# fpgasystems/GPU-FPGA-Recommendation-System

Measured on AMD Instinct MI355X. Metric: inferences/sec at batch 256, higher is better.
Workload: dtype f32; 1 GPU; Model-A (embedding_47_krnl: 47 tables, 1.415 GB) batch=256, fp32 FC 352-1024-512-256-1, all tables resident in one GPU's HBM; hash-filled tables, uniform per-table indices; index rows resident in HBM when the timed region starts (1024 rotating buffers), scores left in HBM (the bench contract's definition of `value`); value_pcie_inclusive = the reference's own loop (cuda_server.c:460-461,494-495): ; batch=256, driver_threads=2, workers_per_thread=2, batches_per_launch=64, parallelism=replicas x1

## Files before the change

### gpu-fpga-recommendation-system_amd/csrc/fr_fused.hip

```cpp
#include "fr_device.h"

#ifdef FR_EPI_FORMS
#include <cstdarg>
#include <cstdio>
thread_local char fr_epi_noted[96];
thread_local int fr_epi_hip_error = 0;
void fr_set_error(const char *, ...) {}
void fr_note_kernel(const char *fmt, ...) {
    va_list ap;
    va_start(ap, fmt);
    vsnprintf(fr_epi_noted, sizeof(fr_epi_noted), fmt, ap);
    va_end(ap);
}
#define FR_NO_DEFAULT_FORM() return FR_ERR_INVALID
#else
static int fused_epi_forward(const FrFusedArgs &a, int kind, hipStream_t s) {
    char name[96] = "";
    const int e = fr_epi_fused_launch(&a, kind, s, name, sizeof(name));
    if (e) FR_FAIL(FR_ERR_HIP, "launch of the epilogue form of the fused kernel failed: %s", hipGetErrorString((hipError_t)e));
    fr_note_kernel("%s", name);
    return FR_OK;
}
#endif

// ... 307 lines not shown
        stamp();
        if (c == 1) wstamp(1);
        ft_gemm_ct<T2W, RB, 32>(acc2, ring2, W2, 32 * T2W * wave, R1, 0, 32 * c, hk, lm);
        if (c == 1) wstamp(2);
        if constexpr (KG > 0) {
            const int cn = (c + 1 < n_chunks) ? c + 1 : c;
            ft_ring_fill<1, RA, KG1>(ring1, W1, cn * 256 + 32 * wave, 0);
        }
    }
    float4 ring3[RA][1];
    ft_ring_fill<1, RA, 32 * T2W>(ring3, W3, 32 * wave, 0);
    __syncthreads();
#pragma unroll
    for (int t = 0; t < T2W; t++) ft_store_tile<EPI>(R2, acc2[t], 32 * (T2W * wave + t), hk, lm, a.epi[1], 32 * (T2W * wave + t));
    __syncthreads();
    stamp();

    f32x16 acc3[1];
#pragma unroll
    for (int i = 0; i < 16; i++) acc3[0][i] = 0.0f;
    ft_gemm_ct<1, RA, 32 * T2W>(acc3, ring3, W3, 32 * wave, R2, 0, 0, hk, lm);
    if (!DB) __syncthreads();
    ft_store_tile<EPI>(R3, acc3[0], 32 * wave, hk, lm, a.epi[2], 32 * wave);
    __syncthreads();
    stamp();
    {
        const int il = tid & 31, sl = tid >> 5;
        const int rows_per = (a.H3 / 4) / 16;
        float s = 0.0f;
        for (int q = sl * rows_per; q < (sl + 1) * rows_per; q++) {
            const uint4 r = R3[(size_t)q * FR_FT_LD + il];
            const float4 w4 = reinterpret_cast<const float4 *>(a.wout)[q];
            s = fmaf(w4.x, __uint_as_float(r.x), s);
            s = fmaf(w4.y, __uint_as_float(r.y), s);
            s = fmaf(w4.z, __uint_as_float(r.z), s);
            s = fmaf(w4.w, __uint_as_float(r.w), s);
        }
        float *part = reinterpret_cast<float *>(R3 + (size_t)64 * FR_FT_LD);
        part[sl * 32 + il] = s;
        __syncthreads();
        if (tid < 32 && m0 + tid < bt.batch) {
            float t = part[tid];
#pragma unroll
            for (int i = 1; i < 16; i++) t += part[i * 32 + tid];
            t = ft_out_bias<EPI>(a, t);
            bt.scores[m0 + tid] = t;
        }
    }
    stamp();
}

#ifndef FR_EPI_FORMS
template <int T2W, int KG, int WPE, bool DB>
__global__ void __launch_bounds__(512, WPE) fr_fused_tile_kernel(const FrFusedArgs a) {
    fused_tile_body<T2W, KG, WPE, DB, false>(a);
}
#else
template <int T2W, int KG, int WPE, bool DB>
__global__ void __launch_bounds__(512, WPE) fr_epi_tile_kernel(const FrFusedArgs a) {
    fused_tile_body<T2W, KG, WPE, DB, true>(a);
}
#endif

size_t frk_fused_lds_bytes(int K, int H2, int wpe) {
    if (wpe == 4) {
        const size_t phase1 = (size_t)(K / 4) + 64, phase2 = (size_t)(H2 / 4) > 68 ? (size_t)(H2 / 4) : 68;
        return (phase1 > phase2 ? phase1 : phase2) * FR_FT_LD * 16;
    }
    const size_t phase1 = (size_t)(K / 4) + 128;
    const size_t phase2 = (size_t)(H2 / 4) + 64 + 4;
    return (phase1 > phase2 ? phase1 : phase2) * FR_FT_LD * 16;
}

bool frk_fused_ok(int K, int H1, int H2, int H3) {
    const bool straight = (K == 352 || K == 880) && H2 == 512;
    if ((!straight && K % 32) || H1 % 256 || (H2 != 256 && H2 != 512) || H3 != 256) return false;
    return frk_fused_lds_bytes(K, H2, 4) <= 160 * 1024;
}

static int fused_wpe(int K, int H2) {
#ifdef FR_EXPERIMENTS
    const int forced = FR_KNOB_ONCE("FUSED_WPE", 0);
    if (forced == 2 || forced == 4) return forced == 4 && frk_fused_lds_bytes(K, H2, 4) > 80 * 1024 ? 2 : forced;
#endif
    return frk_fused_lds_bytes(K, H2, 4) <= 80 * 1024 ? 4 : 2;
}

#ifndef FR_EPI_FORMS
template <int T2W, int KG, int WPE, bool DB>
static int fused_launch_inst(const FrFusedArgs &a, dim3 grid, size_t lds, hipStream_t s) {
    static FrLdsAttrOnce lds_once;
    if (int rc_ = fr_allow_full_lds(&fr_fused_tile_kernel<T2W, KG, WPE, DB>, lds_once)) return rc_;
    fr_fused_tile_kernel<T2W, KG, WPE, DB><<<grid, dim3(512), lds, s>>>(a);
    fr_note_kernel("fr_fused_tile_kernel<%d, %d, %d, %s>", T2W, KG, WPE, DB ? "true" : "false");
    KCHECK();
    return FR_OK;
}

#else
template <int T2W, int KG, int WPE, bool DB>
static int fused_launch_epi_inst(const FrFusedArgs &a, dim3 grid, size_t lds, hipStream_t s) {
    static FrLdsAttrOnce lds_once;
    if (int rc_ = fr_allow_full_lds(&fr_epi_tile_kernel<T2W, KG, WPE, DB>, lds_once)) return rc_;
    fr_epi_tile_kernel<T2W, KG, WPE, DB><<<grid, dim3(512), lds, s>>>(a);
    fr_note_kernel("fr_epi_tile_kernel<%d, %d, %d, %s>", T2W, KG, WPE, DB ? "true" : "false");
    KCHECK();
    return FR_OK;
}

#endif
static bool fused_has_epi(const FrFusedArgs &a) { return a.epi[3].bias != nullptr; }

int frk_fused_launch(const FrFusedArgs &a, hipStream_t s) {
    const int wpe = fused_wpe(a.K, a.H2);
    (void)wpe;
    dim3 grid(a.n_batches * a.tiles_per_batch);
    if (fused_has_epi(a)) {
#ifndef FR_EPI_FORMS
        return fused_epi_forward(a, FR_EPI_KIND_F32, s);
#else
        if (a.H2 == 512 && a.K == 352) return fused_launch_epi_inst<2, 44, 2, true>(a, grid, frk_fused_lds_bytes(a.K, a.H2, 2), s);
        const bool db = frk_fused_lds_bytes(a.K, a.H2, 4) > 80 * 1024 && frk_fused_lds_bytes(a.K, a.H2, 2) <= 160 * 1024;
        const size_t lds = frk_fused_lds_bytes(a.K, a.H2, db ? 2 : 4);
        if (a.H2 == 512) {
            if (a.K == 880) return fused_launch_epi_inst<2, 110, 2, false>(a, grid, lds, s);
            return db ? fused_launch_epi_inst<2, 0, 2, true>(a, grid, lds, s) : fused_launch_epi_inst<2, 0, 2, false>(a, grid, lds, s);
        }
        return db ? fused_launch_epi_inst<1, 0, 2, true>(a, grid, lds, s) : fused_launch_epi_inst<1, 0, 2, false>(a, grid, lds, s);
#endif
    }
#ifdef FR_EPI_FORMS
    FR_NO_DEFAULT_FORM();
#else
    const bool db = wpe == 2 && frk_fused_lds_bytes(a.K, a.H2, 2) <= 160 * 1024;
    const size_t lds = frk_fused_lds_bytes(a.K, a.H2, db ? 2 : 4);
    if (a.H2 == 512) {
        if (a.K == 352) {
#ifdef FR_EXPERIMENTS
            if (wpe != 4) return fused_launch_inst<2, 44, 2, true>(a, grid, lds, s);
#endif
            return fused_launch_inst<2, 44, 4, false>(a, grid, lds, s);
        }
        if (a.K == 880) return fused_launch_inst<2, 110, 2, false>(a, grid, lds, s);
        if (db) return fused_launch_inst<2, 0, 2, true>(a, grid, lds, s);
        return fused_launch_inst<2, 0, 2, false>(a, grid, lds, s);
    }
    if (db) return fused_launch_inst<1, 0, 2, true>(a, grid, lds, s);
    return fused_launch_inst<1, 0, 2, false>(a, grid, lds, s);
#endif
}

constexpr int FR_M2_LD = 65;

template <int NT, int MT, int R, int CNT, int GA, int GB>
__device__ __forceinline__ void ftm_gemm_seg(f32x16 (&acc)[NT][MT], f32x16 (&alt)[MT], float4 (&ring)[R][NT], const FtW &w, int n0, const uint4 *Bq, int gb0,
                                             int g0, int hk, int lm) {
    const unsigned s0 = (unsigned)g0 * w.row2 + (unsigned)n0 * 16u;
    const uint4 *bl = Bq + (size_t)(2 * gb0 + hk) * FR_M2_LD + lm;
    uint4 bcur[MT];
#pragma unroll
    for (int mt = 0; mt < MT; mt++) bcur[mt] = bl[(size_t)(2 * GA) * FR_M2_LD + 32 * mt];
#pragma unroll
    for (int g = GA; g < GB; g++) {
        uint4 bnext[MT];
        const int gn = (g + 1 < GB) ? g + 1 : g;
#pragma unroll
        for (int mt = 0; mt < MT; mt++) bnext[mt] = bl[(size_t)(2 * gn) * FR_M2_LD + 32 * mt];
        const float4(&a4)[NT] = ring[g % R];
#pragma unroll
        for (int c = 0; c < 4; c++)
#pragma unroll
            for (int t = 0; t < NT; t++)
#pragma unroll
                for (int mt = 0; mt < MT; mt++) {
                    const float av = c == 0 ? a4[t].x : c == 1 ? a4[t].y : c == 2 ? a4[t].z : a4[t].w;
                    const uint32_t bv = c == 0 ? bcur[mt].x : c == 1 ? bcur[mt].y : c == 2 ? bcur[mt].z : bcur[mt].w;
                    if (NT == 1 && (c & 1)) alt[mt] = __builtin_amdgcn_mfma_f32_32x32x2f32(av, __uint_as_float(bv), alt[mt], 0, 0, 0);
                    else acc[t][mt] = __builtin_amdgcn_mfma_f32_32x32x2f32(av, __uint_as_float(bv), acc[t][mt], 0, 0, 0);
                }
        if (g + R < CNT) {
#pragma unroll
            for (int t = 0; t < NT; t++) ring[g % R][t] = ft_wload(w, s0 + (unsigned)(g + R) * w.row2, 512 * t);
        }
        __builtin_amdgcn_sched_barrier(0);
#pragma unroll
        for (int mt = 0; mt < MT; mt++) bcur[mt] = bnext[mt];
    }
}

template <int NT, int MT>
__device__ __forceinline__ void ftm_alt_zero(f32x16 (&alt)[MT]) {
    if constexpr (NT == 1) {
#pragma unroll
        for (int mt = 0; mt < MT; mt++)
#pragma unroll
            for (int i = 0; i < 16; i++) alt[mt][i] = 0.0f;
    }
}
template <int NT, int MT>
__device__ __forceinline__ void ftm_alt_add(f32x16 (&acc)[NT][MT], const f32x16 (&alt)[MT]) {
    if constexpr (NT == 1) {
#pragma unroll
        for (int mt = 0; mt < MT; mt++)
#pragma unroll
            for (int i = 0; i < 16; i++) acc[0][mt][i] += alt[mt][i];
    }
}

template <int NT, int MT, int R, int CNT>
__device__ __forceinline__ void ftm_gemm_ct(f32x16 (&acc)[NT][MT], float4 (&ring)[R][NT], const FtW &w, int n0, const uint4 *Bq, int gb0, int g0, int hk,
                                            int lm) {
    f32x16 alt[MT];
    ftm_alt_zero<NT, MT>(alt);
    ftm_gemm_seg<NT, MT, R, CNT, 0, CNT>(acc, alt, ring, w, n0, Bq, gb0, g0, hk, lm);
    ftm_alt_add<NT, MT>(acc, alt);
}

template <bool EPI>
__device__ __forceinline__ void ftm_store_tile(uint4 *img, const f32x16 &acc, int n_local, int m_local, int hk, int lm, const FrEpi &e, int n_glob) {
#pragma unroll
    for (int i = 0; i < 4; i++) {
        float c0 = acc[4 * i + 0], c1 = acc[4 * i + 1], c2 = acc[4 * i + 2], c3 = acc[4 * i + 3];
        ft_epi4<EPI>(c0, c1, c2, c3, e, n_glob + 8 * i, hk);
        uint4 v;
        v.x = __float_as_uint(c0);
        v.y = __float_as_uint(c1);
        v.z = __float_as_uint(c2);
        v.w = __float_as_uint(c3);
        img[(size_t)((n_local >> 2) + 2 * i + hk) * FR_M2_LD + m_local + lm] = v;
    }
}

template <int W0, int W>
struct FtmSlot {
    static constexpr int IPT = W / 8;
    uint64_t base;
    uint32_t stride, rows, icol;
    bool dense;
    uint32_t id[IPT];
    uint4 v[IPT];
    static __device__ __forceinline__ int word(int lane) { return W0 + (lane & (W - 1)); }
    static __device__ __forceinline__ int item(int lane, int wave, int i) { return lane / W + (64 / W) * (wave + 8 * i); }
    __device__ __forceinline__ void desc(const FrFusedArgs &a, const FrFusedBatch &bt, int lane) {
        const int w = word(lane) < a.n_words ? word(lane) : a.n_words - 1;
        const uint4 d0 = reinterpret_cast<const uint4 *>(a.words)[2 * w];
        const uint4 d1 = reinterpret_cast<const uint4 *>(a.words)[2 * w + 1];
        dense = (d0.w & FR_DESC_DENSE) != 0;
        base = (dense ? (uint64_t)reinterpret_cast<uintptr_t>(bt.dense) : 0ull) + (((uint64_t)d0.y << 32) | d0.x);
        stride = d0.z, rows = d1.x, icol = dense ? 0u : d0.w * 4u;
    }
    __device__ __forceinline__ void index(const FrFusedArgs &a, const __amdgpu_buffer_rsrc_t &rs_idx, int m0, int lane, int wave) {
#pragma unroll
        for (int i = 0; i < IPT; i++)
            id[i] = (uint32_t)__builtin_amdgcn_raw_buffer_load_b32(rs_idx, (unsigned)(m0 + item(lane, wave, i)) * (unsigned)a.idx_stride * 4u + icol, 0, 0);
    }
    __device__ __forceinline__ bool check(const FrFusedBatch &bt, int m0, int lane, int wave) {
        bool bad = false;
#pragma unroll
        for (int i = 0; i < IPT; i++) {
            const unsigned m = (unsigned)(m0 + item(lane, wave, i));
            uint32_t r = id[i];
            const bool oob = !dense & (r >= rows);
            bad |= oob;
            r = oob ? 0u : r;
            id[i] = dense ? (m < (unsigned)bt.batch ? m : 0u) : r;
        }
        return bad;
    }
    __device__ __forceinline__ void load() {
#pragma unroll
        for (int i = 0; i < IPT; i++) {
            typedef const u32x4_t __attribute__((address_space(1))) * gptr_t;
            const u32x4_t q = *(gptr_t)(base + (uint64_t)id[i] * stride);
            v[i] = make_uint4(q.x, q.y, q.z, q.w);
        }
    }
    __device__ __forceinline__ void put(const FrFusedArgs &a, const FrFusedBatch &bt, uint4 *Xq, int m0, int lane, int wave) const {
        if (word(lane) < a.n_words) {
#pragma unroll
            for (int i = 0; i < IPT; i++) {
                const int it = item(lane, wave, i);
                Xq[(size_t)word(lane) * FR_M2_LD + it] = (m0 + it < bt.batch) ? v[i] : make_uint4(0u, 0u, 0u, 0u);
            }
        }
    }
};
template <class... S>
struct FtmSlice : S... {
    __device__ __forceinline__ void desc(const FrFusedArgs &a, const FrFusedBatch &bt, int lane) { (S::desc(a, bt, lane), ...); }
    __device__ __forceinline__ void index(const FrFusedArgs &a, const __amdgpu_buffer_rsrc_t &rs, int m0, int lane, int wave) { (S::index(a, rs, m0, lane, wave), ...); }
    __device__ __forceinline__ bool check(const FrFusedBatch &bt, int m0, int lane, int wave) { return (false | ... | S::check(bt, m0, lane, wave)); }
    __device__ __forceinline__ void load() { (S::load(), ...); }
    __device__ __forceinline__ void put(const FrFusedArgs &a, const FrFusedBatch &bt, uint4 *Xq, int m0, int lane, int wave) const { (S::put(a, bt, Xq, m0, lane, wave), ...); }
};
constexpr int FR_M2_CUT1 = 12, FR_M2_CUT2 = 28;
using FtmS0 = FtmSlice<FtmSlot<0, 16>, FtmSlot<16, 8>>;
using FtmS1 = FtmSlice<FtmSlot<24, 32>>;
using FtmS2 = FtmSlice<FtmSlot<56, 32>>;

template <int KG, bool EPI>
__device__ __forceinline__ void fused_tile_m2_body(const FrFusedArgs &a) {
    extern __shared__ uint4 lds[];
    constexpr int LD = FR_M2_LD, MT = 2, T2W = 2, TI = 64;
    constexpr int RA = 12, RB = 8, GC1 = FR_M2_CUT1, GC2 = FR_M2_CUT2;
    static_assert(KG == 44 && GC1 < GC2 && GC2 < KG, "the slices above are cut for 88 record words");
    const int KQ = a.K / 4;
    uint4 *Xq = lds;
    uint4 *R1 = Xq + (size_t)KQ * LD;
    uint4 *R2 = lds;
    uint4 *R3 = lds;
    const int tid = threadIdx.x, lane = tid & 63;
    const int wave = __builtin_amdgcn_readfirstlane(tid >> 6);
    const int hk = lane >> 5, lm = lane & 31;
    const int bi = blockIdx.x / a.tiles_per_batch, tile = blockIdx.x - bi * a.tiles_per_batch;
    const FrFusedBatch &bt = a.b[bi];
    const int m0 = tile * TI;
    if (m0 >= bt.batch) return;
    const FtW W1 = ft_w(a.w1q, a.K, a.H1, hk, lm), W2 = ft_w(a.w2q, a.H1, a.H2, hk, lm), W3 = ft_w(a.w3q, a.H2, a.H3, hk, lm);
    float4 ring1[RA][1];
    ft_ring_fill<1, RA, KG>(ring1, W1, 32 * wave, 0);

    FtmS0 s0;
    FtmS1 s1;
    FtmS2 s2;
    s0.desc(a, bt, lane), s1.desc(a, bt, lane), s2.desc(a, bt, lane);
    const __amdgpu_buffer_rsrc_t rs_idx = __builtin_amdgcn_make_buffer_rsrc(const_cast<int32_t *>(bt.idx), 0, (unsigned)bt.batch * (unsigned)a.idx_stride * 4u, 0x00020000);
    s0.index(a, rs_idx, m0, lane, wave), s1.index(a, rs_idx, m0, lane, wave), s2.index(a, rs_idx, m0, lane, wave);
    const bool bad0 = s0.check(bt, m0, lane, wave), bad1 = s1.check(bt, m0, lane, wave), bad2 = s2.check(bt, m0, lane, wave);
    s0.load(), s1.load();
    if (bad0 | bad1 | bad2) atomicOr_system(a.err_flag, 1);
    s0.put(a, bt, Xq, m0, lane, wave);
    __syncthreads();

    const int n_chunks = a.H1 / 256;
    f32x16 acc2[T2W][MT];
    auto fc2_chunk = [&](int c, f32x16(&acc1)[1][MT]) {
        float4 ring2[RB][T2W];
        ft_ring_fill<T2W, RB, 32>(ring2, W2, 32 * T2W * wave, 32 * c);
        if (c > 0) __syncthreads();
#pragma unroll
        for (int mt = 0; mt < MT; mt++) ftm_store_tile<EPI>(R1, acc1[0][mt], 32 * wave, 32 * mt, hk, lm, a.epi[0], c * 256 + 32 * wave);
        __syncthreads();
        ftm_gemm_ct<T2W, MT, RB, 32>(acc2, ring2, W2, 32 * T2W * wave, R1, 0, 32 * c, hk, lm);
        if constexpr (EPI) {
            const int cn = (c + 1 < n_chunks) ? c + 1 : c;
            ft_ring_fill<1, RA, KG>(ring1, W1, cn * 256 + 32 * wave, 0);
        } else {
            if (c + 1 < n_chunks) ft_ring_fill<1, RA, KG>(ring1, W1, (c + 1) * 256 + 32 * wave, 0);
            else ft_ring_fill<1, RA, 32 * T2W>(ring1, W3, 32 * wave, 0);
        }
    };
    {
        f32x16 acc1[1][MT], alt1[MT];
#pragma unroll
        for (int mt = 0; mt < MT; mt++)
#pragma unroll
            for (int i = 0; i < 16; i++) acc1[0][mt][i] = 0.0f;
        ftm_alt_zero<1, MT>(alt1);
        ftm_gemm_seg<1, MT, RA, KG, 0, GC1>(acc1, alt1, ring1, W1, 32 * wave, Xq, 0, 0, hk, lm);
        s1.put(a, bt, Xq, m0, lane, wave);
        __syncthreads();
        s2.load();
        ftm_gemm_seg<1, MT, RA, KG, GC1, GC2>(acc1, alt1, ring1, W1, 32 * wave, Xq, 0, 0, hk, lm);
        s2.put(a, bt, Xq, m0, lane, wave);
        __syncthreads();
        ftm_gemm_seg<1, MT, RA, KG, GC2, KG>(acc1, alt1, ring1, W1, 32 * wave, Xq, 0, 0, hk, lm);
        ftm_alt_add<1, MT>(acc1, alt1);
#pragma unroll
        for (int t = 0; t < T2W; t++)
#pragma unroll
            for (int mt = 0; mt < MT; mt++)
#pragma unroll
                for (int i = 0; i < 16; i++) acc2[t][mt][i] = 0.0f;
        fc2_chunk(0, acc1);
    }
    for (int c = 1; c < n_chunks; c++) {
        f32x16 acc1[1][MT];
#pragma unroll
        for (int mt = 0; mt < MT; mt++)
#pragma unroll
            for (int i = 0; i < 16; i++) acc1[0][mt][i] = 0.0f;
        ftm_gemm_ct<1, MT, RA, KG>(acc1, ring1, W1, c * 256 + 32 * wave, Xq, 0, 0, hk, lm);
        fc2_chunk(c, acc1);
    }
    float4(&ring3)[RA][1] = ring1;
    if constexpr (EPI) ft_ring_fill<1, RA, 32 * T2W>(ring3, W3, 32 * wave, 0);
    __syncthreads();
#pragma unroll
    for (int t = 0; t < T2W; t++)
#pragma unroll
        for (int mt = 0; mt < MT; mt++) ftm_store_tile<EPI>(R2, acc2[t][mt], 32 * (T2W * wave + t), 32 * mt, hk, lm, a.epi[1], 32 * (T2W * wave + t));
    __syncthreads();

    f32x16 acc3[1][MT];
#pragma unroll
    for (int mt = 0; mt < MT; mt++)
#pragma unroll
        for (int i = 0; i < 16; i++) acc3[0][mt][i] = 0.0f;
    ftm_gemm_ct<1, MT, RA, 32 * T2W>(acc3, ring3, W3, 32 * wave, R2, 0, 0, hk, lm);
    __syncthreads();
#pragma unroll
    for (int mt = 0; mt < MT; mt++) ftm_store_tile<EPI>(R3, acc3[0][mt], 32 * wave, 32 * mt, hk, lm, a.epi[2], 32 * wave);
    __syncthreads();
    {
        const int il = tid & 63, sg = tid >> 6;
        const int rows_per = (a.H3 / 4) / 16;
        float *part = reinterpret_cast<float *>(R3 + (size_t)(a.H3 / 4) * LD);
#pragma unroll
        for (int h2 = 0; h2 < 2; h2++) {
            const int sl = 2 * sg + h2;
            float s = 0.0f;
            for (int q = sl * rows_per; q < (sl + 1) * rows_per; q++) {
                const uint4 r = R3[(size_t)q * LD + il];
                const float4 w4 = reinterpret_cast<const float4 *>(a.wout)[q];
                s = fmaf(w4.x, __uint_as_float(r.x), s);
                s = fmaf(w4.y, __uint_as_float(r.y), s);
                s = fmaf(w4.z, __uint_as_float(r.z), s);
                s = fmaf(w4.w, __uint_as_float(r.w), s);
            }
            part[sl * 64 + il] = s;
        }
        __syncthreads();
        if (tid < 64 && m0 + tid < bt.batch) {
            float t = part[tid];
#pragma unroll
            for (int i = 1; i < 16; i++) t += part[i * 64 + tid];
            t = ft_out_bias<EPI>(a, t);
            bt.scores[m0 + tid] = t;
        }
    }
}

#ifndef FR_EPI_FORMS
template <int KG>
__global__ void __launch_bounds__(512) fr_fused_tile_m2_kernel(const FrFusedArgs a) {
    fused_tile_m2_body<KG, false>(a);
}
#else
template <int KG>
__global__ void __launch_bounds__(512) fr_epi_tile_m2_kernel(const FrFusedArgs a) {
    fused_tile_m2_body<KG, true>(a);
}
#endif

bool frk_fused_m2_ok(int K, int H1, int H2, int H3) { return K == 352 && H1 % 256 == 0 && H2 == 512 && H3 == 256; }

int frk_fused_m2_launch(const FrFusedArgs &a, hipStream_t s) {
    static FrLdsAttrOnce lds_once;
    const size_t rows1 = (size_t)(a.K / 4) + 64, rows2 = (size_t)(a.H2 / 4), rows3 = 64 + 4;
    const size_t rows = rows1 > rows2 ? (rows1 > rows3 ? rows1 : rows3) : (rows2 > rows3 ? rows2 : rows3);
#ifdef FR_EPI_FORMS
    if (!fused_has_epi(a)) FR_NO_DEFAULT_FORM();
    if (int rc_ = fr_allow_full_lds(&fr_epi_tile_m2_kernel<44>, lds_once)) return rc_;
    fr_epi_tile_m2_kernel<44><<<dim3(a.n_batches * a.tiles_per_batch), dim3(512), rows * FR_M2_LD * 16, s>>>(a);
    fr_note_kernel("fr_epi_tile_m2_kernel<44>");
#else
    if (fused_has_epi(a)) return fused_epi_forward(a, FR_EPI_KIND_F32_M2, s);
    if (int rc_ = fr_allow_full_lds(&fr_fused_tile_m2_kernel<44>, lds_once)) return rc_;
    fr_fused_tile_m2_kernel<44><<<dim3(a.n_batches * a.tiles_per_batch), dim3(512), rows * FR_M2_LD * 16, s>>>(a);
    fr_note_kernel("fr_fused_tile_m2_kernel<44>");
#endif
    KCHECK();
    return FR_OK;
}

template <int NT, int MT, int R, int CNT>
__device__ __forceinline__ void fth_gemm_ct(f32x16 (&acc)[NT][MT], const FtW &w, int n0, const uint4 *Bh, int ld, int gb0, int g0, int hk, int lm) {
    const unsigned s0 = (unsigned)g0 * w.row2 + (unsigned)n0 * 16u;
    const uint4 *bl = Bh + (size_t)(2 * gb0 + hk) * ld + lm;
    uint4 ring[R][NT];
#pragma unroll
    for (int g = 0; g < R && g < CNT; g++)
#pragma unroll
        for (int t = 0; t < NT; t++) ring[g][t] = __builtin_bit_cast(uint4, ft_wload(w, s0 + (unsigned)g * w.row2, 512 * t));
#pragma unroll
    for (int g = 0; g < CNT; g++) {
        uint4 b8[MT];
#pragma unroll
        for (int mt = 0; mt < MT; mt++) b8[mt] = bl[(size_t)(2 * g) * ld + 32 * mt];
#pragma unroll
        for (int t = 0; t < NT; t++)
#pragma unroll
            for (int mt = 0; mt < MT; mt++)
                acc[t][mt] = __builtin_amdgcn_mfma_f32_32x32x16_bf16(__builtin_bit_cast(bf16x8, ring[g % R][t]), __builtin_bit_cast(bf16x8, b8[mt]),
                                                                     acc[t][mt], 0, 0, 0);
        if (g + R < CNT) {
#pragma unroll
            for (int t = 0; t < NT; t++) ring[g % R][t] = __builtin_bit_cast(uint4, ft_wload(w, s0 + (unsigned)(g + R) * w.row2, 512 * t));
        }
        __builtin_amdgcn_sched_barrier(0);
    }
}

template <bool EPI>
__device__ __forceinline__ void fth_store_tile(uint4 *img, int ld, const f32x16 &acc, int n_local, int m_local, int hk, int lm, const FrEpi &e, int n_glob) {
    uint2 *h = reinterpret_cast<uint2 *>(img);
#pragma unroll
    for (int i = 0; i < 4; i++) {
        float c0 = acc[4 * i + 0], c1 = acc[4 * i + 1], c2 = acc[4 * i + 2], c3 = acc[4 * i + 3];
        ft_epi4<EPI>(c0, c1, c2, c3, e, n_glob + 8 * i, hk);
        uint2 v;
        v.x = pack_bf16x2(c0, c1);
        v.y = pack_bf16x2(c2, c3);
        h[((size_t)((n_local >> 3) + i) * ld + m_local + lm) * 2 + hk] = v;
    }
}

template <int MT, int T2W, int KG, bool DB, int RD, int PD, bool EPI>
__device__ __forceinline__ void fused_tile_h_body(const FrFusedArgs &a) {
    extern __shared__ uint4 lds[];
    constexpr int LD = 32 * MT + 1, TI = 32 * MT;
    const int KO = a.K / 8;
    uint4 *Xh = lds;
    uint4 *R1b[2] = {Xh + (size_t)KO * LD, Xh + (size_t)(KO + (DB ? 32 : 0)) * LD};
    uint4 *R2 = lds;
    uint4 *R3 = lds + (size_t)(a.H2 / 8) * LD;
    const int tid = threadIdx.x, lane = tid & 63;
    const int wave = __builtin_amdgcn_readfirstlane(tid >> 6);
    const int hk = lane >> 5, lm = lane & 31;
    const int bi = blockIdx.x / a.tiles_per_batch, tile = blockIdx.x - bi * a.tiles_per_batch;
    const FrFusedBatch &bt = a.b[bi];
    const int m0 = tile * TI;
    if (m0 >= bt.batch) return;
    int n_st = 0;
    auto stamp = [&]() {
        if (a.stamps && lane == 0 && n_st < 14) {
            a.stamps[16ull * (8ull * blockIdx.x + wave) + n_st] = __builtin_amdgcn_s_memrealtime();
            if (n_st == 1) a.stamps[16ull * (8ull * blockIdx.x + wave) + 14] = __builtin_amdgcn_s_memtime();
            if (n_st == 9) a.stamps[16ull * (8ull * blockIdx.x + wave) + 15] = __builtin_amdgcn_s_memtime();
        }
        n_st++;
    };
    stamp();

    {
        const int wl = tid & 63, ig = tid >> 6;
        constexpr int IPT = TI / 8, NB = (4 * KG + 63) / 64;
        uint2 *Xh2 = reinterpret_cast<uint2 *>(Xh);
        const bool bad = ft_gather_tile<NB, IPT>(a, bt, m0, wl, ig, [&](int w, int i, const uint4 &x) {
            uint2 hv;
            hv.x = pack_bf16x2(__uint_as_float(x.x), __uint_as_float(x.y));
            hv.y = pack_bf16x2(__uint_as_float(x.z), __uint_as_float(x.w));
            Xh2[((size_t)(w >> 1) * LD + IPT * ig + i) * 2 + (w & 1)] = hv;
        });
        if (bad) atomicOr_system(a.err_flag, 1);
    }
    __syncthreads();
    stamp();

    f32x16 acc2[T2W][MT];
#pragma unroll
    for (int t = 0; t < T2W; t++)
#pragma unroll
        for (int mt = 0; mt < MT; mt++)
#pragma unroll
            for (int i = 0; i < 16; i++) acc2[t][mt][i] = 0.0f;
    const int n_chunks = a.H1 / 256;
    const FtW W1 = ft_w(a.w1q, a.K / 2, a.H1, hk, lm), W2 = ft_w(a.w2q, a.H1 / 2, a.H2, hk, lm), W3 = ft_w(a.w3q, a.H2 / 2, a.H3, hk, lm);
    static_assert(T2W == 2 && KG >= RD && RD >= 8 && RD <= 32 && RD % 2 == 0, "the stream ring assumes two n tiles per wave in FC2 (32 elements per chunk) and at least RD k groups in FC1");
    constexpr int OFF2 = KG % RD;
    uint4 ring[RD];
    auto w1load = [&](int c, int g) { return __builtin_bit_cast(uint4, ft_wload(W1, (unsigned)g * W1.row2 + (unsigned)(c * 256 + 32 * wave) * 16u, 0)); };
    auto w2load = [&](int c, int e) {
        return __builtin_bit_cast(uint4, ft_wload(W2, (unsigned)(16 * c + (e >> 1)) * W2.row2 + (unsigned)(32 * T2W * wave) * 16u, 512 * (e & 1)));
    };
#pragma unroll
    for (int g = 0; g < RD; g++) ring[g] = w1load(0, g);
    const uint4 *blx = Xh + (size_t)hk * LD + lm;
    static_assert(PD == 1 || PD == 2 || PD == 4, "B ring: 16 % PD must be 0");
    uint4 bq[PD][MT];
#pragma unroll
    for (int i = 0; i < PD; i++)
#pragma unroll
        for (int mt = 0; mt < MT; mt++) bq[i][mt] = blx[(size_t)(2 * i) * LD + 32 * mt];
    for (int c = 0; c < n_chunks; c++) {
        f32x16 acc1[1][MT];
#pragma unroll
        for (int mt = 0; mt < MT; mt++)
#pragma unroll
            for (int i = 0; i < 16; i++) acc1[0][mt][i] = 0.0f;
#pragma unroll
        for (int g = 0; g < KG; g++) {
#pragma unroll
// ... 376 lines not shown
```

Before: 70.55 million inferences/s.

## Interleave next-chunk weight prefetch into FC2 GEMM and preload output weights

```diff
diff --git a/gpu-fpga-recommendation-system_amd/csrc/fr_fused.hip b/gpu-fpga-recommendation-system_amd/csrc/fr_fused.hip
--- a/gpu-fpga-recommendation-system_amd/csrc/fr_fused.hip
+++ b/gpu-fpga-recommendation-system_amd/csrc/fr_fused.hip
@@ -483,9 +483,12 @@
 
 constexpr int FR_M2_LD = 65;
 
-template <int NT, int MT, int R, int CNT, int GA, int GB>
+struct FtmNothingUnder {
+    __device__ __forceinline__ void operator()(int) const {}
+};
+template <int NT, int MT, int R, int CNT, int GA, int GB, class Under = FtmNothingUnder>
 __device__ __forceinline__ void ftm_gemm_seg(f32x16 (&acc)[NT][MT], f32x16 (&alt)[MT], float4 (&ring)[R][NT], const FtW &w, int n0, const uint4 *Bq, int gb0,
-                                             int g0, int hk, int lm) {
+                                             int g0, int hk, int lm, Under &&under = Under()) {
     const unsigned s0 = (unsigned)g0 * w.row2 + (unsigned)n0 * 16u;
     const uint4 *bl = Bq + (size_t)(2 * gb0 + hk) * FR_M2_LD + lm;
     uint4 bcur[MT];
@@ -513,6 +516,7 @@
 #pragma unroll
             for (int t = 0; t < NT; t++) ring[g % R][t] = ft_wload(w, s0 + (unsigned)(g + R) * w.row2, 512 * t);
         }
+        under(g);
         __builtin_amdgcn_sched_barrier(0);
 #pragma unroll
         for (int mt = 0; mt < MT; mt++) bcur[mt] = bnext[mt];
@@ -562,6 +566,10 @@
     }
 }
 
+struct FtmRecord {
+    const struct FrWordDesc *words;
+    int n_words, idx_stride;
+};
 template <int W0, int W>
 struct FtmSlot {
     static constexpr int IPT = W / 8;
@@ -572,7 +580,7 @@
     uint4 v[IPT];
     static __device__ __forceinline__ int word(int lane) { return W0 + (lane & (W - 1)); }
     static __device__ __forceinline__ int item(int lane, int wave, int i) { return lane / W + (64 / W) * (wave + 8 * i); }
-    __device__ __forceinline__ void desc(const FrFusedArgs &a, const FrFusedBatch &bt, int lane) {
+    __device__ __forceinline__ void desc(const FtmRecord &a, const FrFusedBatch &bt, int lane) {
         const int w = word(lane) < a.n_words ? word(lane) : a.n_words - 1;
         const uint4 d0 = reinterpret_cast<const uint4 *>(a.words)[2 * w];
         const uint4 d1 = reinterpret_cast<const uint4 *>(a.words)[2 * w + 1];
@@ -580,7 +588,7 @@
         base = (dense ? (uint64_t)reinterpret_cast<uintptr_t>(bt.dense) : 0ull) + (((uint64_t)d0.y << 32) | d0.x);
         stride = d0.z, rows = d1.x, icol = dense ? 0u : d0.w * 4u;
     }
-    __device__ __forceinline__ void index(const FrFusedArgs &a, const __amdgpu_buffer_rsrc_t &rs_idx, int m0, int lane, int wave) {
+    __device__ __forceinline__ void index(const FtmRecord &a, const __amdgpu_buffer_rsrc_t &rs_idx, int m0, int lane, int wave) {
 #pragma unroll
         for (int i = 0; i < IPT; i++)
             id[i] = (uint32_t)__builtin_amdgcn_raw_buffer_load_b32(rs_idx, (unsigned)(m0 + item(lane, wave, i)) * (unsigned)a.idx_stride * 4u + icol, 0, 0);
@@ -606,7 +614,7 @@
             v[i] = make_uint4(q.x, q.y, q.z, q.w);
         }
     }
-    __device__ __forceinline__ void put(const FrFusedArgs &a, const FrFusedBatch &bt, uint4 *Xq, int m0, int lane, int wave) const {
+    __device__ __forceinline__ void put(const FtmRecord &a, const FrFusedBatch &bt, uint4 *Xq, int m0, int lane, int wave) const {
         if (word(lane) < a.n_words) {
 #pragma unroll
             for (int i = 0; i < IPT; i++) {
@@ -618,11 +626,11 @@
 };
 template <class... S>
 struct FtmSlice : S... {
-    __device__ __forceinline__ void desc(const FrFusedArgs &a, const FrFusedBatch &bt, int lane) { (S::desc(a, bt, lane), ...); }
-    __device__ __forceinline__ void index(const FrFusedArgs &a, const __amdgpu_buffer_rsrc_t &rs, int m0, int lane, int wave) { (S::index(a, rs, m0, lane, wave), ...); }
+    __device__ __forceinline__ void desc(const FtmRecord &a, const FrFusedBatch &bt, int lane) { (S::desc(a, bt, lane), ...); }
+    __device__ __forceinline__ void index(const FtmRecord &a, const __amdgpu_buffer_rsrc_t &rs, int m0, int lane, int wave) { (S::index(a, rs, m0, lane, wave), ...); }
     __device__ __forceinline__ bool check(const FrFusedBatch &bt, int m0, int lane, int wave) { return (false | ... | S::check(bt, m0, lane, wave)); }
     __device__ __forceinline__ void load() { (S::load(), ...); }
-    __device__ __forceinline__ void put(const FrFusedArgs &a, const FrFusedBatch &bt, uint4 *Xq, int m0, int lane, int wave) const { (S::put(a, bt, Xq, m0, lane, wave), ...); }
+    __device__ __forceinline__ void put(const FtmRecord &a, const FrFusedBatch &bt, uint4 *Xq, int m0, int lane, int wave) const { (S::put(a, bt, Xq, m0, lane, wave), ...); }
 };
 constexpr int FR_M2_CUT1 = 12, FR_M2_CUT2 = 28;
 using FtmS0 = FtmSlice<FtmSlot<0, 16>, FtmSlot<16, 8>>;
@@ -635,7 +643,13 @@
     constexpr int LD = FR_M2_LD, MT = 2, T2W = 2, TI = 64;
     constexpr int RA = 12, RB = 8, GC1 = FR_M2_CUT1, GC2 = FR_M2_CUT2;
     static_assert(KG == 44 && GC1 < GC2 && GC2 < KG, "the slices above are cut for 88 record words");
-    const int KQ = a.K / 4;
+    int tiles_per_batch = a.tiles_per_batch, K = a.K, H1 = a.H1, H2 = a.H2, H3 = a.H3;
+    FtmRecord rec = {a.words, a.n_words, a.idx_stride};
+    const float4 *w1q = a.w1q, *w2q = a.w2q, *w3q = a.w3q;
+    const float *wout = a.wout;
+    asm volatile("" : "+s"(tiles_per_batch), "+s"(K), "+s"(H1), "+s"(H2), "+s"(H3), "+s"(rec.n_words), "+s"(rec.idx_stride), "+s"(w1q), "+s"(w2q), "+s"(w3q), "+s"(wout)
+                 : "s"(rec.words));
+    const int KQ = K / 4;
     uint4 *Xq = lds;
     uint4 *R1 = Xq + (size_t)KQ * LD;
     uint4 *R2 = lds;
@@ -643,27 +657,28 @@
     const int tid = threadIdx.x, lane = tid & 63;
     const int wave = __builtin_amdgcn_readfirstlane(tid >> 6);
     const int hk = lane >> 5, lm = lane & 31;
-    const int bi = blockIdx.x / a.tiles_per_batch, tile = blockIdx.x - bi * a.tiles_per_batch;
-    const FrFusedBatch &bt = a.b[bi];
+    const int bi = blockIdx.x / tiles_per_batch, tile = blockIdx.x - bi * tiles_per_batch;
+    FrFusedBatch bt = a.b[bi];
+    asm volatile("" : "+s"(bt.idx), "+s"(bt.dense), "+s"(bt.scores), "+s"(bt.batch));
     const int m0 = tile * TI;
     if (m0 >= bt.batch) return;
-    const FtW W1 = ft_w(a.w1q, a.K, a.H1, hk, lm), W2 = ft_w(a.w2q, a.H1, a.H2, hk, lm), W3 = ft_w(a.w3q, a.H2, a.H3, hk, lm);
+    const FtW W1 = ft_w(w1q, K, H1, hk, lm), W2 = ft_w(w2q, H1, H2, hk, lm), W3 = ft_w(w3q, H2, H3, hk, lm);
     float4 ring1[RA][1];
     ft_ring_fill<1, RA, KG>(ring1, W1, 32 * wave, 0);
 
     FtmS0 s0;
     FtmS1 s1;
     FtmS2 s2;
-    s0.desc(a, bt, lane), s1.desc(a, bt, lane), s2.desc(a, bt, lane);
-    const __amdgpu_buffer_rsrc_t rs_idx = __builtin_amdgcn_make_buffer_rsrc(const_cast<int32_t *>(bt.idx), 0, (unsigned)bt.batch * (unsigned)a.idx_stride * 4u, 0x00020000);
-    s0.index(a, rs_idx, m0, lane, wave), s1.index(a, rs_idx, m0, lane, wave), s2.index(a, rs_idx, m0, lane, wave);
+    s0.desc(rec, bt, lane), s1.desc(rec, bt, lane), s2.desc(rec, bt, lane);
+    const __amdgpu_buffer_rsrc_t rs_idx = __builtin_amdgcn_make_buffer_rsrc(const_cast<int32_t *>(bt.idx), 0, (unsigned)bt.batch * (unsigned)rec.idx_stride * 4u, 0x00020000);
+    s0.index(rec, rs_idx, m0, lane, wave), s1.index(rec, rs_idx, m0, lane, wave), s2.index(rec, rs_idx, m0, lane, wave);
     const bool bad0 = s0.check(bt, m0, lane, wave), bad1 = s1.check(bt, m0, lane, wave), bad2 = s2.check(bt, m0, lane, wave);
     s0.load(), s1.load();
     if (bad0 | bad1 | bad2) atomicOr_system(a.err_flag, 1);
-    s0.put(a, bt, Xq, m0, lane, wave);
-    __syncthreads();
-
-    const int n_chunks = a.H1 / 256;
+    s0.put(rec, bt, Xq, m0, lane, wave);
+    __syncthreads();
+
+    const int n_chunks = H1 / 256;
     f32x16 acc2[T2W][MT];
     auto fc2_chunk = [&](int c, f32x16(&acc1)[1][MT]) {
         float4 ring2[RB][T2W];
@@ -672,14 +687,16 @@
 #pragma unroll
         for (int mt = 0; mt < MT; mt++) ftm_store_tile<EPI>(R1, acc1[0][mt], 32 * wave, 32 * mt, hk, lm, a.epi[0], c * 256 + 32 * wave);
         __syncthreads();
-        ftm_gemm_ct<T2W, MT, RB, 32>(acc2, ring2, W2, 32 * T2W * wave, R1, 0, 32 * c, hk, lm);
-        if constexpr (EPI) {
-            const int cn = (c + 1 < n_chunks) ? c + 1 : c;
-            ft_ring_fill<1, RA, KG>(ring1, W1, cn * 256 + 32 * wave, 0);
-        } else {
-            if (c + 1 < n_chunks) ft_ring_fill<1, RA, KG>(ring1, W1, (c + 1) * 256 + 32 * wave, 0);
-            else ft_ring_fill<1, RA, 32 * T2W>(ring1, W3, 32 * wave, 0);
-        }
+        const bool to_fc3 = c + 1 >= n_chunks;
+        FtW Wn;
+        Wn.rs = to_fc3 ? W3.rs : W1.rs;
+        Wn.voff = to_fc3 ? W3.voff : W1.voff;
+        Wn.row2 = to_fc3 ? W3.row2 : W1.row2;
+        const unsigned sn = (unsigned)((to_fc3 ? 0 : (c + 1) * 256) + 32 * wave) * 16u;
+        f32x16 none[MT];
+        ftm_gemm_seg<T2W, MT, RB, 32, 0, 32>(acc2, none, ring2, W2, 32 * T2W * wave, R1, 0, 32 * c, hk, lm, [&](int g) {
+            if (g >= 32 - RA) ring1[g - (32 - RA)][0] = ft_wload(Wn, sn + (unsigned)(g - (32 - RA)) * Wn.row2, 0);
+        });
     };
     {
         f32x16 acc1[1][MT], alt1[MT];
@@ -689,11 +706,11 @@
             for (int i = 0; i < 16; i++) acc1[0][mt][i] = 0.0f;
         ftm_alt_zero<1, MT>(alt1);
         ftm_gemm_seg<1, MT, RA, KG, 0, GC1>(acc1, alt1, ring1, W1, 32 * wave, Xq, 0, 0, hk, lm);
-        s1.put(a, bt, Xq, m0, lane, wave);
+        s1.put(rec, bt, Xq, m0, lane, wave);
         __syncthreads();
         s2.load();
         ftm_gemm_seg<1, MT, RA, KG, GC1, GC2>(acc1, alt1, ring1, W1, 32 * wave, Xq, 0, 0, hk, lm);
-        s2.put(a, bt, Xq, m0, lane, wave);
+        s2.put(rec, bt, Xq, m0, lane, wave);
         __syncthreads();
         ftm_gemm_seg<1, MT, RA, KG, GC2, KG>(acc1, alt1, ring1, W1, 32 * wave, Xq, 0, 0, hk, lm);
         ftm_alt_add<1, MT>(acc1, alt1);
@@ -715,7 +732,22 @@
         fc2_chunk(c, acc1);
     }
     float4(&ring3)[RA][1] = ring1;
-    if constexpr (EPI) ft_ring_fill<1, RA, 32 * T2W>(ring3, W3, 32 * wave, 0);
+    constexpr int Q3 = 64, ROWS_PER = Q3 / 16;
+    float4 wo[2][ROWS_PER];
+    float out_bias = 0.0f;
+    const __amdgpu_buffer_rsrc_t rs_wout = __builtin_amdgcn_make_buffer_rsrc(const_cast<float *>(wout), 0, (unsigned)Q3 * 16u, 0x00020000);
+#pragma unroll
+    for (int h2 = 0; h2 < 2; h2++)
+#pragma unroll
+        for (int j = 0; j < ROWS_PER; j++) {
+            const u32x4 v = __builtin_amdgcn_raw_buffer_load_b128(rs_wout, 0, (unsigned)((2 * wave + h2) * ROWS_PER + j) * 16u, 0);
+            wo[h2][j] = make_float4(__uint_as_float(v.x), __uint_as_float(v.y), __uint_as_float(v.z), __uint_as_float(v.w));
+        }
+    if constexpr (EPI) {
+        out_bias = *(const float __attribute__((address_space(4))) *)(uintptr_t)a.epi[3].bias;
+        asm volatile("" : "+s"(out_bias));
+    }
+    __builtin_amdgcn_sched_barrier(0);
     __syncthreads();
 #pragma unroll
     for (int t = 0; t < T2W; t++)
@@ -734,16 +766,16 @@
     for (int mt = 0; mt < MT; mt++) ftm_store_tile<EPI>(R3, acc3[0][mt], 32 * wave, 32 * mt, hk, lm, a.epi[2], 32 * wave);
     __syncthreads();
     {
-        const int il = tid & 63, sg = tid >> 6;
-        const int rows_per = (a.H3 / 4) / 16;
-        float *part = reinterpret_cast<float *>(R3 + (size_t)(a.H3 / 4) * LD);
+        const int il = tid & 63;
+        float *part = reinterpret_cast<float *>(R3 + (size_t)Q3 * LD);
 #pragma unroll
         for (int h2 = 0; h2 < 2; h2++) {
-            const int sl = 2 * sg + h2;
+            const int sl = 2 * wave + h2;
             float s = 0.0f;
-            for (int q = sl * rows_per; q < (sl + 1) * rows_per; q++) {
-                const uint4 r = R3[(size_t)q * LD + il];
-                const float4 w4 = reinterpret_cast<const float4 *>(a.wout)[q];
+#pragma unroll
+            for (int j = 0; j < ROWS_PER; j++) {
+                const uint4 r = R3[(size_t)(sl * ROWS_PER + j) * LD + il];
+                const float4 w4 = wo[h2][j];
                 s = fmaf(w4.x, __uint_as_float(r.x), s);
                 s = fmaf(w4.y, __uint_as_float(r.y), s);
                 s = fmaf(w4.z, __uint_as_float(r.z), s);
@@ -756,8 +788,9 @@
             float t = part[tid];
 #pragma unroll
             for (int i = 1; i < 16; i++) t += part[i * 64 + tid];
-            t = ft_out_bias<EPI>(a, t);
-            bt.scores[m0 + tid] = t;
+            if constexpr (EPI) t += out_bias;
+            typedef float __attribute__((address_space(1))) * gfloat_t;
+            ((gfloat_t)bt.scores)[m0 + tid] = t;
         }
     }
 }
```

Result: no change. 70.56 million inferences/s (median of 2 runs) (+0.0%).

## Skew layer boundaries in fused m2 kernel to overlap stores, barriers and next-layer GEMM

Applied to the files above, without the earlier changes.

```diff
diff --git a/gpu-fpga-recommendation-system_amd/csrc/fr_fused.hip b/gpu-fpga-recommendation-system_amd/csrc/fr_fused.hip
--- a/gpu-fpga-recommendation-system_amd/csrc/fr_fused.hip
+++ b/gpu-fpga-recommendation-system_amd/csrc/fr_fused.hip
@@ -483,40 +483,93 @@
 
 constexpr int FR_M2_LD = 65;
 
-template <int NT, int MT, int R, int CNT, int GA, int GB>
+constexpr int FR_M2_NO_STAMP = -1;
+#ifdef FR_M2_DIAG
+struct FtmDiag {
+    __amdgpu_buffer_rsrc_t rs;
+    unsigned voff;
+    __device__ __forceinline__ void init(const FrFusedArgs &a, int lane, int wave) {
+        rs = __builtin_amdgcn_make_buffer_rsrc(a.stamps, 0, a.stamps ? gridDim.x * 1024u : 0u, 0x00020000);
+        voff = (lane == 0 && (wave & 3) == 0) ? (2u * blockIdx.x + (unsigned)(wave >> 2)) * 512u : 0xFFFFF000u;
+    }
+    __device__ __forceinline__ void put(int slot, unsigned long long t) const {
+        typedef unsigned u32x2_t __attribute__((ext_vector_type(2)));
+        u32x2_t v;
+        v.x = (unsigned)t, v.y = (unsigned)(t >> 32);
+        __builtin_amdgcn_raw_buffer_store_b64(v, rs, voff, (unsigned)(slot & 63) * 8u, 0);
+    }
+    __device__ __forceinline__ void stamp(int slot) const {
+        if (slot == FR_M2_NO_STAMP) return;
+        __builtin_amdgcn_sched_barrier(0);
+        put(slot, __builtin_amdgcn_s_memtime());
+        __builtin_amdgcn_sched_barrier(0);
+    }
+    __device__ __forceinline__ void stamp_after(int slot, uint32_t dep) const {
+        if (slot == FR_M2_NO_STAMP) return;
+        __builtin_amdgcn_sched_barrier(0);
+        asm volatile("" ::"v"(dep));
+        stamp(slot);
+    }
+    __device__ __forceinline__ void realtime(int slot) const { put(slot, __builtin_amdgcn_s_memrealtime()); }
+};
+#else
+struct FtmDiag {
+    __device__ __forceinline__ void init(const FrFusedArgs &, int, int) {}
+    __device__ __forceinline__ void stamp(int) const {}
+    __device__ __forceinline__ void stamp_after(int, uint32_t) const {}
+    __device__ __forceinline__ void realtime(int) const {}
+};
+#endif
+constexpr __device__ __forceinline__ int ftm_edge_slot(int e, int p) { return 1 + 3 * e + p; }
+
+struct FtmNoHook {
+    __device__ __forceinline__ void operator()(int) const {}
+};
+template <int NT, int MT, int R, int CNT, int GA, int GB, int M0 = 0, int M1 = MT, bool REFILL = true, class Hook = FtmNoHook>
 __device__ __forceinline__ void ftm_gemm_seg(f32x16 (&acc)[NT][MT], f32x16 (&alt)[MT], float4 (&ring)[R][NT], const FtW &w, int n0, const uint4 *Bq, int gb0,
-                                             int g0, int hk, int lm) {
+                                             int g0, int hk, int lm, const FtmDiag &dg = FtmDiag(), int st_first = FR_M2_NO_STAMP,
+                                             int st_last = FR_M2_NO_STAMP, const Hook &after_group = Hook()) {
+    static_assert(0 <= M0 && M0 < M1 && M1 <= MT && GA < GB && GB <= CNT, "a segment runs at least one group of at least one item tile");
     const unsigned s0 = (unsigned)g0 * w.row2 + (unsigned)n0 * 16u;
     const uint4 *bl = Bq + (size_t)(2 * gb0 + hk) * FR_M2_LD + lm;
     uint4 bcur[MT];
 #pragma unroll
-    for (int mt = 0; mt < MT; mt++) bcur[mt] = bl[(size_t)(2 * GA) * FR_M2_LD + 32 * mt];
+    for (int mt = M0; mt < M1; mt++) bcur[mt] = bl[(size_t)(2 * GA) * FR_M2_LD + 32 * mt];
+    dg.stamp_after(st_first, bcur[M1 - 1].x);
 #pragma unroll
     for (int g = GA; g < GB; g++) {
         uint4 bnext[MT];
         const int gn = (g + 1 < GB) ? g + 1 : g;
 #pragma unroll
-        for (int mt = 0; mt < MT; mt++) bnext[mt] = bl[(size_t)(2 * gn) * FR_M2_LD + 32 * mt];
+        for (int mt = M0; mt < M1; mt++) bnext[mt] = bl[(size_t)(2 * gn) * FR_M2_LD + 32 * mt];
         const float4(&a4)[NT] = ring[g % R];
 #pragma unroll
         for (int c = 0; c < 4; c++)
 #pragma unroll
             for (int t = 0; t < NT; t++)
 #pragma unroll
-                for (int mt = 0; mt < MT; mt++) {
+                for (int mt = M0; mt < M1; mt++) {
                     const float av = c == 0 ? a4[t].x : c == 1 ? a4[t].y : c == 2 ? a4[t].z : a4[t].w;
                     const uint32_t bv = c == 0 ? bcur[mt].x : c == 1 ? bcur[mt].y : c == 2 ? bcur[mt].z : bcur[mt].w;
                     if (NT == 1 && (c & 1)) alt[mt] = __builtin_amdgcn_mfma_f32_32x32x2f32(av, __uint_as_float(bv), alt[mt], 0, 0, 0);
                     else acc[t][mt] = __builtin_amdgcn_mfma_f32_32x32x2f32(av, __uint_as_float(bv), acc[t][mt], 0, 0, 0);
                 }
-        if (g + R < CNT) {
+        if (REFILL && g + R < CNT) {
 #pragma unroll
             for (int t = 0; t < NT; t++) ring[g % R][t] = ft_wload(w, s0 + (unsigned)(g + R) * w.row2, 512 * t);
         }
+        after_group(g);
         __builtin_amdgcn_sched_barrier(0);
 #pragma unroll
-        for (int mt = 0; mt < MT; mt++) bcur[mt] = bnext[mt];
-    }
+        for (int mt = M0; mt < M1; mt++) bcur[mt] = bnext[mt];
+    }
+    dg.stamp(st_last);
+}
+
+__device__ __forceinline__ void ftm_barrier() {
+    __builtin_amdgcn_sched_barrier(0);
+    __syncthreads();
+    __builtin_amdgcn_sched_barrier(0);
 }
 
 template <int NT, int MT>
@@ -540,10 +593,10 @@
 
 template <int NT, int MT, int R, int CNT>
 __device__ __forceinline__ void ftm_gemm_ct(f32x16 (&acc)[NT][MT], float4 (&ring)[R][NT], const FtW &w, int n0, const uint4 *Bq, int gb0, int g0, int hk,
-                                            int lm) {
+                                            int lm, const FtmDiag &dg = FtmDiag(), int st_first = FR_M2_NO_STAMP, int st_last = FR_M2_NO_STAMP) {
     f32x16 alt[MT];
     ftm_alt_zero<NT, MT>(alt);
-    ftm_gemm_seg<NT, MT, R, CNT, 0, CNT>(acc, alt, ring, w, n0, Bq, gb0, g0, hk, lm);
+    ftm_gemm_seg<NT, MT, R, CNT, 0, CNT>(acc, alt, ring, w, n0, Bq, gb0, g0, hk, lm, dg, st_first, st_last);
     ftm_alt_add<NT, MT>(acc, alt);
 }
 
@@ -625,6 +678,9 @@
     __device__ __forceinline__ void put(const FrFusedArgs &a, const FrFusedBatch &bt, uint4 *Xq, int m0, int lane, int wave) const { (S::put(a, bt, Xq, m0, lane, wave), ...); }
 };
 constexpr int FR_M2_CUT1 = 12, FR_M2_CUT2 = 28;
+#ifndef FR_M2_SKEW
+#define FR_M2_SKEW 4
+#endif
 using FtmS0 = FtmSlice<FtmSlot<0, 16>, FtmSlot<16, 8>>;
 using FtmS1 = FtmSlice<FtmSlot<24, 32>>;
 using FtmS2 = FtmSlice<FtmSlot<56, 32>>;
@@ -634,7 +690,8 @@
     extern __shared__ uint4 lds[];
     constexpr int LD = FR_M2_LD, MT = 2, T2W = 2, TI = 64;
     constexpr int RA = 12, RB = 8, GC1 = FR_M2_CUT1, GC2 = FR_M2_CUT2;
-    static_assert(KG == 44 && GC1 < GC2 && GC2 < KG, "the slices above are cut for 88 record words");
+    constexpr int SK = FR_M2_SKEW, GF = 12;
+    static_assert(KG == 44 && GC1 < GC2 && GC2 < KG - SK && GF < KG - SK && 1 < SK && SK <= RB, "the slices above are cut for 88 record words");
     const int KQ = a.K / 4;
     uint4 *Xq = lds;
     uint4 *R1 = Xq + (size_t)KQ * LD;
@@ -648,6 +705,10 @@
     const int m0 = tile * TI;
     if (m0 >= bt.batch) return;
     const FtW W1 = ft_w(a.w1q, a.K, a.H1, hk, lm), W2 = ft_w(a.w2q, a.H1, a.H2, hk, lm), W3 = ft_w(a.w3q, a.H2, a.H3, hk, lm);
+    FtmDiag dg;
+    dg.init(a, lane, wave);
+    dg.realtime(33);
+    dg.stamp(0);
     float4 ring1[RA][1];
     ft_ring_fill<1, RA, KG>(ring1, W1, 32 * wave, 0);
 
@@ -665,21 +726,27 @@
 
     const int n_chunks = a.H1 / 256;
     f32x16 acc2[T2W][MT];
-    auto fc2_chunk = [&](int c, f32x16(&acc1)[1][MT]) {
-        float4 ring2[RB][T2W];
-        ft_ring_fill<T2W, RB, 32>(ring2, W2, 32 * T2W * wave, 32 * c);
-        if (c > 0) __syncthreads();
-#pragma unroll
-        for (int mt = 0; mt < MT; mt++) ftm_store_tile<EPI>(R1, acc1[0][mt], 32 * wave, 32 * mt, hk, lm, a.epi[0], c * 256 + 32 * wave);
-        __syncthreads();
-        ftm_gemm_ct<T2W, MT, RB, 32>(acc2, ring2, W2, 32 * T2W * wave, R1, 0, 32 * c, hk, lm);
-        if constexpr (EPI) {
-            const int cn = (c + 1 < n_chunks) ? c + 1 : c;
-            ft_ring_fill<1, RA, KG>(ring1, W1, cn * 256 + 32 * wave, 0);
-        } else {
-            if (c + 1 < n_chunks) ft_ring_fill<1, RA, KG>(ring1, W1, (c + 1) * 256 + 32 * wave, 0);
-            else ft_ring_fill<1, RA, 32 * T2W>(ring1, W3, 32 * wave, 0);
-        }
+    float4 ring2[RB][T2W];
+    f32x16 none[MT];
+    auto chunk_tail = [&](int c, f32x16(&acc1)[1][MT], f32x16(&alt1)[MT]) {
+        const int n1 = c * 256 + 32 * wave, n2 = 32 * T2W * wave;
+        ftm_gemm_seg<1, MT, RA, KG, KG - SK, KG, 0, 1>(acc1, alt1, ring1, W1, n1, Xq, 0, 0, hk, lm);
+        ft_ring_fill<T2W, RB, 32>(ring2, W2, n2, 32 * c);
+        ftm_gemm_seg<1, MT, RA, KG, KG - SK, KG - SK + 1, 1, 2>(acc1, alt1, ring1, W1, n1, Xq, 0, 0, hk, lm);
+#pragma unroll
+        for (int i = 0; i < 16; i++) acc1[0][0][i] += alt1[0][i];
+        ftm_store_tile<EPI>(R1, acc1[0][0], 32 * wave, 0, hk, lm, a.epi[0], n1);
+        ftm_gemm_seg<1, MT, RA, KG, KG - SK + 1, KG, 1, 2>(acc1, alt1, ring1, W1, n1, Xq, 0, 0, hk, lm, dg, FR_M2_NO_STAMP, ftm_edge_slot(2 * c, 0));
+        ftm_barrier();
+        dg.stamp(ftm_edge_slot(2 * c, 1));
+        ftm_gemm_seg<T2W, MT, RB, 32, 0, 1, 0, 1, false>(acc2, none, ring2, W2, n2, R1, 0, 32 * c, hk, lm, dg, ftm_edge_slot(2 * c, 2));
+#pragma unroll
+        for (int i = 0; i < 16; i++) acc1[0][1][i] += alt1[1][i];
+        ftm_store_tile<EPI>(R1, acc1[0][1], 32 * wave, 32, hk, lm, a.epi[0], n1);
+        ftm_gemm_seg<T2W, MT, RB, 32, 1, SK, 0, 1, false>(acc2, none, ring2, W2, n2, R1, 0, 32 * c, hk, lm);
+        ftm_barrier();
+        ftm_gemm_seg<T2W, MT, RB, 32, 0, SK, 1, 2>(acc2, none, ring2, W2, n2, R1, 0, 32 * c, hk, lm);
+        ftm_gemm_seg<T2W, MT, RB, 32, SK, 32 - RB>(acc2, none, ring2, W2, n2, R1, 0, 32 * c, hk, lm);
     };
     {
         f32x16 acc1[1][MT], alt1[MT];
@@ -695,44 +762,66 @@
         ftm_gemm_seg<1, MT, RA, KG, GC1, GC2>(acc1, alt1, ring1, W1, 32 * wave, Xq, 0, 0, hk, lm);
         s2.put(a, bt, Xq, m0, lane, wave);
         __syncthreads();
-        ftm_gemm_seg<1, MT, RA, KG, GC2, KG>(acc1, alt1, ring1, W1, 32 * wave, Xq, 0, 0, hk, lm);
-        ftm_alt_add<1, MT>(acc1, alt1);
+        ftm_gemm_seg<1, MT, RA, KG, GC2, KG - SK>(acc1, alt1, ring1, W1, 32 * wave, Xq, 0, 0, hk, lm);
 #pragma unroll
         for (int t = 0; t < T2W; t++)
 #pragma unroll
             for (int mt = 0; mt < MT; mt++)
 #pragma unroll
                 for (int i = 0; i < 16; i++) acc2[t][mt][i] = 0.0f;
-        fc2_chunk(0, acc1);
+        chunk_tail(0, acc1, alt1);
     }
     for (int c = 1; c < n_chunks; c++) {
-        f32x16 acc1[1][MT];
+        const unsigned s1 = (unsigned)(c * 256 + 32 * wave) * 16u;
+        ftm_gemm_seg<T2W, MT, RB, 32, 32 - RB, 32>(acc2, none, ring2, W2, 32 * T2W * wave, R1, 0, 32 * (c - 1), hk, lm, dg, FR_M2_NO_STAMP, ftm_edge_slot(2 * c - 1, 0),
+                                                   [&](int g) {
+                                                       const int j = 2 * (g - (32 - RB));
+                                                       if (j < RA) ring1[j][0] = ft_wload(W1, s1 + (unsigned)j * W1.row2, 0);
+                                                       if (j + 1 < RA) ring1[j + 1][0] = ft_wload(W1, s1 + (unsigned)(j + 1) * W1.row2, 0);
+                                                   });
+        f32x16 acc1[1][MT], alt1[MT];
 #pragma unroll
         for (int mt = 0; mt < MT; mt++)
 #pragma unroll
             for (int i = 0; i < 16; i++) acc1[0][mt][i] = 0.0f;
-        ftm_gemm_ct<1, MT, RA, KG>(acc1, ring1, W1, c * 256 + 32 * wave, Xq, 0, 0, hk, lm);
-        fc2_chunk(c, acc1);
+        ftm_alt_zero<1, MT>(alt1);
+        ftm_gemm_seg<1, MT, RA, KG, 0, GF>(acc1, alt1, ring1, W1, c * 256 + 32 * wave, Xq, 0, 0, hk, lm, dg, ftm_edge_slot(2 * c - 1, 2));
+        ftm_barrier();
+        ftm_gemm_seg<1, MT, RA, KG, GF, KG - SK>(acc1, alt1, ring1, W1, c * 256 + 32 * wave, Xq, 0, 0, hk, lm);
+        chunk_tail(c, acc1, alt1);
     }
     float4(&ring3)[RA][1] = ring1;
-    if constexpr (EPI) ft_ring_fill<1, RA, 32 * T2W>(ring3, W3, 32 * wave, 0);
-    __syncthreads();
-#pragma unroll
-    for (int t = 0; t < T2W; t++)
-#pragma unroll
-        for (int mt = 0; mt < MT; mt++) ftm_store_tile<EPI>(R2, acc2[t][mt], 32 * (T2W * wave + t), 32 * mt, hk, lm, a.epi[1], 32 * (T2W * wave + t));
-    __syncthreads();
-
-    f32x16 acc3[1][MT];
+    const int n2 = 32 * T2W * wave, gl = 32 * (n_chunks - 1);
+    ftm_gemm_seg<T2W, MT, RB, 32, 32 - RB, 32 - SK>(acc2, none, ring2, W2, n2, R1, 0, gl, hk, lm);
+    ftm_gemm_seg<T2W, MT, RB, 32, 32 - SK, 32, 0, 1>(acc2, none, ring2, W2, n2, R1, 0, gl, hk, lm);
+    ft_ring_fill<1, RA, 32 * T2W>(ring3, W3, 32 * wave, 0);
+    ftm_barrier();
+    ftm_gemm_seg<T2W, MT, RB, 32, 32 - SK, 32 - SK + 1, 1, 2>(acc2, none, ring2, W2, n2, R1, 0, gl, hk, lm);
+#pragma unroll
+    for (int t = 0; t < T2W; t++) ftm_store_tile<EPI>(R2, acc2[t][0], 32 * (T2W * wave + t), 0, hk, lm, a.epi[1], 32 * (T2W * wave + t));
+    ftm_gemm_seg<T2W, MT, RB, 32, 32 - SK + 1, 32, 1, 2>(acc2, none, ring2, W2, n2, R1, 0, gl, hk, lm, dg, FR_M2_NO_STAMP, ftm_edge_slot(2 * n_chunks - 1, 0));
+    ftm_barrier();
+    dg.stamp(ftm_edge_slot(2 * n_chunks - 1, 1));
+
+    f32x16 acc3[1][MT], alt3[MT];
 #pragma unroll
     for (int mt = 0; mt < MT; mt++)
 #pragma unroll
         for (int i = 0; i < 16; i++) acc3[0][mt][i] = 0.0f;
-    ftm_gemm_ct<1, MT, RA, 32 * T2W>(acc3, ring3, W3, 32 * wave, R2, 0, 0, hk, lm);
+    ftm_alt_zero<1, MT>(alt3);
+    ftm_gemm_seg<1, MT, RA, 32 * T2W, 0, 1, 0, 1, false>(acc3, alt3, ring3, W3, 32 * wave, R2, 0, 0, hk, lm, dg, ftm_edge_slot(2 * n_chunks - 1, 2));
+#pragma unroll
+    for (int t = 0; t < T2W; t++) ftm_store_tile<EPI>(R2, acc2[t][1], 32 * (T2W * wave + t), 32, hk, lm, a.epi[1], 32 * (T2W * wave + t));
+    ftm_gemm_seg<1, MT, RA, 32 * T2W, 1, SK, 0, 1, false>(acc3, alt3, ring3, W3, 32 * wave, R2, 0, 0, hk, lm);
+    ftm_barrier();
+    ftm_gemm_seg<1, MT, RA, 32 * T2W, 0, SK, 1, 2>(acc3, alt3, ring3, W3, 32 * wave, R2, 0, 0, hk, lm);
+    ftm_gemm_seg<1, MT, RA, 32 * T2W, SK, 32 * T2W>(acc3, alt3, ring3, W3, 32 * wave, R2, 0, 0, hk, lm, dg, FR_M2_NO_STAMP, ftm_edge_slot(8, 0));
+    ftm_alt_add<1, MT>(acc3, alt3);
     __syncthreads();
 #pragma unroll
     for (int mt = 0; mt < MT; mt++) ftm_store_tile<EPI>(R3, acc3[0][mt], 32 * wave, 32 * mt, hk, lm, a.epi[2], 32 * wave);
     __syncthreads();
+    dg.stamp(ftm_edge_slot(8, 1));
     {
         const int il = tid & 63, sg = tid >> 6;
         const int rows_per = (a.H3 / 4) / 16;
@@ -752,6 +841,7 @@
             part[sl * 64 + il] = s;
         }
         __syncthreads();
+        dg.stamp(ftm_edge_slot(9, 1));
         if (tid < 64 && m0 + tid < bt.batch) {
             float t = part[tid];
 #pragma unroll
@@ -760,6 +850,9 @@
             bt.scores[m0 + tid] = t;
         }
     }
+    dg.stamp(31);
+    dg.stamp(32);
+    dg.realtime(34);
 }
 
 #ifndef FR_EPI_FORMS
```

New measurement: 70.11 million inferences/s before, 70.55 million inferences/s after (median of 2 runs). No clear change (+0.6%).
